# inferrna/Core

Hardware: AMD Instinct MI355X
Metric: Mrays/s (primary+shadow), 1M-tri scene (higher is better)
Workload: dtype f32

## Files before the change

core_amd/csrc/yk_device.hip:

```cpp
#include <hip/hip_runtime.h>

#include <algorithm>
#include <atomic>
#include <climits>
#include <chrono>
#include <cmath>
#include <cstdio>
#include <cstdlib>
#include <cstring>
#include <mutex>
#include <type_traits>
#include <stdexcept>
#include <string>
#include <thread>
#include <vector>

#include "../../include/yk_api.h"
#include "../../include/yk_test_hooks.h"
#include "../../include/yk_test_hooks_light.h"
#include "../../include/yk_test_hooks_camera.h"
#include "../../include/yk_test_hooks_film.h"
#include "../../include/yk_test_hooks_depth.h"
#include "photon_map.h"
#include "scene.h"
// ... 2665 lines not shown
          B.scol_next[3 * c + 1] = sc.g;
          B.scol_next[3 * c + 2] = sc.b;
          ps |= PS_CONT;
        }
      }
      B.pstate[c] = ps;
    }
  }
  unsigned sbase, qn;
  wave_append2<YK_BOUNCE_APPEND_WAVE>(qword, valid ? (unsigned)nr : 0u, emit_next ? 1u : 0u, sbase, qn);
  if (valid) flush_shadow(B, c, kend, nr, sbase + qpre, traced);
  if (emit_next) {
    st_ray(&B.q_rays[qin ^ 1][qn], nxt);
    B.q_owner[qin ^ 1][qn] = (int)c;
  }
}

inline auto shade_primary_fn(bool diff, bool xl, bool ao) {
  if (ao)
    return xl ? (diff ? k_shade_primary<true, true, true> : k_shade_primary<false, true, true>)
              : (diff ? k_shade_primary<true, false, true> : k_shade_primary<false, false, true>);
  return xl ? (diff ? k_shade_primary<true, true, false> : k_shade_primary<false, true, false>)
            : (diff ? k_shade_primary<true, false, false> : k_shade_primary<false, false, false>);
}
inline auto shade_bounce_fn(bool diff, bool xl) {
  return xl ? (diff ? k_shade_bounce<true, true> : k_shade_bounce<false, true>)
            : (diff ? k_shade_bounce<true, false> : k_shade_bounce<false, false>);
}

__global__ void __launch_bounds__(256) k_resolve_bounce(Batch B, RenderConst R,
                                                        const unsigned long long* __restrict__ qin_word, int depth,
                                                        int qin) {
  const long long nq = (long long)(*qin_word >> 32);
  const long long qi = (long long)blockIdx.x * blockDim.x + threadIdx.x;
  if (qi >= nq) return;
  const long long c = B.q_owner[qin][qi];
  const int ps = B.pstate[c];
  if (!(ps & PS_RESOLVE)) return;
  c3 lcol = C3(0.f, 0.f, 0.f);
  if (ps & PS_EST) {
    const int lnum = R.nlights > 1 ? B.lsel[c] : 0;
    lcol = cscale((float)R.nlights, resolve_light(B, c, 0, lnum));
  }
  if ((depth == 1 || R.spec) && (ps & PS_EMIT))
    lcol = cadd(lcol, C3(B.emit_b[3 * c], B.emit_b[3 * c + 1], B.emit_b[3 * c + 2]));
  const c3 thr = C3(B.thr[3 * c], B.thr[3 * c + 1], B.thr[3 * c + 2]);
  B.pathcol[3 * c] = B.pathcol[3 * c] + lcol.r * thr.r;
  B.pathcol[3 * c + 1] = B.pathcol[3 * c + 1] + lcol.g * thr.g;
  B.pathcol[3 * c + 2] = B.pathcol[3 * c + 2] + lcol.b * thr.b;
  if (ps & PS_CONT) {
    B.thr[3 * c] = thr.r * B.scol_next[3 * c];
    B.thr[3 * c + 1] = thr.g * B.scol_next[3 * c + 1];
    B.thr[3 * c + 2] = thr.b * B.scol_next[3 * c + 2];
    B.pstate[c] = PS_ALIVE;
  } else {
    B.pstate[c] = 0;
  }
}


__host__ __device__ inline Batch merged_region(Batch B, int depth) {
  B.slot_base = (long long)depth * B.cap;
  B.mq_region = depth;
  if (depth >= 1) {
    const long long o = (long long)(depth - 1) * B.cap;
    B.pstate += o;
    B.lsel += o;
    B.emit_b += 3 * o;
    B.scol_next += 3 * o;
  }
  return B;
}

__global__ void __launch_bounds__(256) k_resolve_merged(Batch B, RenderConst R, long long nc, int bounces) {
  const long long c = (long long)blockIdx.x * blockDim.x + threadIdx.x;
  if (c >= nc) return;
  c3 col = C3(B.col[3 * c], B.col[3 * c + 1], B.col[3 * c + 2]);
  if (!(B.prim_hit[c] & PH_DIFFUSE)) {
    B.samples[c] = make_float4(col.r, col.g, col.b, B.alpha[c]);
    return;
  }
  {
    c3 dl = C3(0.f, 0.f, 0.f);
    int k0 = 0;
    for (int l = 0; l < R.nlights; ++l) {
      dl = cadd(dl, resolve_light(B, c, k0, l));
      k0 += c_lights[l].nslots;
    }
    col = C3(col.r + dl.r, col.g + dl.g, col.b + dl.b);
  }
  c3 thr = C3(B.thr[3 * c], B.thr[3 * c + 1], B.thr[3 * c + 2]);
  c3 pc = C3(0.f, 0.f, 0.f);
  for (int depth = 1; depth <= bounces; ++depth) {
    const Batch Bd = merged_region(B, depth);
    const int ps = Bd.pstate[c];
    if (!(ps & PS_RESOLVE)) break;
    c3 lcol = C3(0.f, 0.f, 0.f);
    if (ps & PS_EST) {
      const int lnum = R.nlights > 1 ? Bd.lsel[c] : 0;
      lcol = cscale((float)R.nlights, resolve_light(Bd, c, 0, lnum));
    }
    if (depth == 1 && (ps & PS_EMIT))
      lcol = cadd(lcol, C3(Bd.emit_b[3 * c], Bd.emit_b[3 * c + 1], Bd.emit_b[3 * c + 2]));
    pc = C3(pc.r + lcol.r * thr.r, pc.g + lcol.g * thr.g, pc.b + lcol.b * thr.b);
    if (!(ps & PS_CONT)) break;
    thr = C3(thr.r * Bd.scol_next[3 * c], thr.g * Bd.scol_next[3 * c + 1], thr.b * Bd.scol_next[3 * c + 2]);
  }
  const float ns = (float)R.nsub;
  col = cadd(col, C3(pc.r / ns, pc.g / ns, pc.b / ns));
  B.samples[c] = make_float4(col.r, col.g, col.b, B.alpha[c]);
}

__global__ void __launch_bounds__(256) k_finish(Batch B, RenderConst R, long long nc) {
  const long long c = (long long)blockIdx.x * blockDim.x + threadIdx.x;
  if (c >= nc) return;
  c3 col = C3(B.col[3 * c], B.col[3 * c + 1], B.col[3 * c + 2]);
  if (R.integrator == YK_INTEGRATOR_PATH && (B.prim_hit[c] & PH_DIFFUSE)) {
    const float ns = (float)R.nsub;
    col = cadd(col, C3(B.pathcol[3 * c] / ns, B.pathcol[3 * c + 1] / ns, B.pathcol[3 * c + 2] / ns));
  }
  B.samples[c] = make_float4(col.r, col.g, col.b, B.alpha[c]);
}


enum : int { NF_HIT = 1, NF_LIGHT = 2, NF_LOOP = 4, NF_LOOPT = 8, NF_SPEC = 16 };

struct NodeStore {
  float* E;
  float* D;
  float* P;
  int* flags;
  int* child;
  float* rcol;
  float* alpha;
  yk_ray* ray;
  unsigned* soffs;
  unsigned* psample;
  unsigned long long* count;
  long long cap;
  int* overflow;
  float* malpha;
};

__global__ void __launch_bounds__(256) k_finish_spec(Batch B, RenderConst R, NodeStore NS, long long base,
                                                     long long n) {
  const long long i = (long long)blockIdx.x * blockDim.x + threadIdx.x;
  if (i >= n) return;
  const long long node = base + i;
  const int ph = B.prim_hit[i];
  const bool loop = R.integrator == YK_INTEGRATOR_PATH && (ph & PH_DIFFUSE);
  c3 P = C3(0.f, 0.f, 0.f);
  if (loop) {
    const float ns = (float)R.nsub;
    P = C3(B.pathcol[3 * i] / ns, B.pathcol[3 * i + 1] / ns, B.pathcol[3 * i + 2] / ns);
  }
  int f = 0;
  if (ph & PH_HIT) f |= NF_HIT;
  if (ph & PH_LIGHT) f |= NF_LIGHT;
  if (loop) f |= NF_LOOP | (B.incl[i] ? NF_LOOPT : 0);
  NS.flags[node] = f;
#pragma unroll
  for (int k = 0; k < 3; ++k) {
    NS.E[3 * node + k] = (ph & PH_HIT) ? B.emit0[3 * i + k] : 0.f;
    NS.D[3 * node + k] = B.col[3 * i + k];
  }
  NS.P[3 * node] = P.r;
  NS.P[3 * node + 1] = P.g;
  NS.P[3 * node + 2] = P.b;
  NS.child[2 * node] = -1;
  NS.child[2 * node + 1] = -1;
  NS.malpha[node] = 1.f;
  if (R.level == 0) NS.alpha[node] = B.alpha[i];
}

__global__ void __launch_bounds__(256) k_spawn(DScene S, Batch B, RenderConst R, NodeStore NS, long long base,
                                               long long n) {
  const long long i = (long long)blockIdx.x * blockDim.x + threadIdx.x;
  if (i >= n || !(B.prim_hit[i] & PH_HIT)) return;
  const int lv = R.level + 1;
  if (lv > R.rdepth || lv >= 20) return;
  const yk_hit h = B.p_hits[i];
  const yk_ray r = B.p_rays[i];
  const v3 from = V3(r.from[0], r.from[1], r.from[2]), dir = V3(r.dir[0], r.dir[1], r.dir[2]);
  const SurfPt sp = make_surface(S, from, dir, h);
  const DMat& M = c_mats[sp.mat];
  if (!(M.flags & (BSDF_SPECULAR | BSDF_FILTER))) return;
  const long long node = base + i;
  NS.flags[node] |= NF_SPEC;
  if (R.integrator == YK_INTEGRATOR_PHOTON && (M.flags & BSDF_FILTER)) {
    const v3 wo = vneg(dir);
    const float Kr = mat_fresnel(M, wo, face_forward(sp.Ng, sp.N, wo));
    const float refl = (1.f - M.comp[0] * Kr) * M.comp[1];
    NS.malpha[node] = 1.f - refl;
  }
  bool refl, refr;
  v3 d[2];
  c3 col[2];
  mat_specular(M, sp, vneg(dir), refl, refr, d, col);
  const bool want[2] = {refl, refr};
#pragma unroll
  for (int k = 0; k < 2; ++k) {
    if (!want[k]) continue;
    const unsigned long long id = atomicAdd(NS.count, 1ull);
    if ((long long)id >= NS.cap) {
      *NS.overflow = 1;
      continue;
    }
    NS.child[2 * node + k] = (int)id;
    NS.rcol[6 * node + 3 * k] = col[k].r;
    NS.rcol[6 * node + 3 * k + 1] = col[k].g;
    NS.rcol[6 * node + 3 * k + 2] = col[k].b;
    put_ray(NS.ray[id], sp.P, d[k], YK_MIN_RAYDIST, -1.0f);
    NS.soffs[id] = B.soffs[i];
    NS.psample[id] = B.psample[i];
  }
}

__global__ void __launch_bounds__(256) k_fold(Batch B, RenderConst R, NodeStore NS, long long nc) {
  const long long c = (long long)blockIdx.x * blockDim.x + threadIdx.x;
  if (c >= nc) return;
  constexpr int kMaxLevel = 22;
  int nodes[kMaxLevel], stage[kMaxLevel];
  c3 acc[kMaxLevel];
  float alp[kMaxLevel];
  const bool pt = R.integrator == YK_INTEGRATOR_PATH, pm = R.integrator == YK_INTEGRATOR_PHOTON;
  const float a_init = R.transp_bg ? 0.f : 1.f;
  float result_alpha = 0.f;
  bool e = true;
  int dd = 0;
  nodes[0] = (int)c;
  stage[0] = 0;
  c3 result = C3(0.f, 0.f, 0.f);
  for (;;) {
    const int n = nodes[dd];
    const int F = NS.flags[n];
    if (stage[dd] == 0) {
      c3 col = C3(NS.D[3 * n], NS.D[3 * n + 1], NS.D[3 * n + 2]);
      if (F & NF_HIT) {
        if (dd == 0) e = true;
        const bool incl = pt ? e : true;
        const c3 E = ((F & NF_LIGHT) && !incl) ? C3(0.f, 0.f, 0.f)
                                               : C3(NS.E[3 * n], NS.E[3 * n + 1], NS.E[3 * n + 2]);
        col = cadd(E, col);
        col = cadd(col, C3(NS.P[3 * n], NS.P[3 * n + 1], NS.P[3 * n + 2]));
        if (pt && (F & NF_LOOP)) e = (F & NF_LOOPT) != 0;
        if (F & NF_SPEC) e = true;
      }
      acc[dd] = col;
      alp[dd] = a_init;
      stage[dd] = 1;
      const int ch = (F & NF_HIT) ? NS.child[2 * n] : -1;
      if (ch >= 0 && dd + 1 < kMaxLevel) {
        ++dd;
        nodes[dd] = ch;
        stage[dd] = 0;
        continue;
      }
    }
    if (stage[dd] == 1) {
      stage[dd] = 2;
      const int ch = (F & NF_HIT) ? NS.child[2 * n + 1] : -1;
      if (ch >= 0 && dd + 1 < kMaxLevel) {
        ++dd;
        nodes[dd] = ch;
        stage[dd] = 0;
        continue;
      }
    }
    const c3 v = acc[dd];
    const float m = NS.malpha[n];
    const float va = (F & NF_HIT) ? m + (1.f - m) * alp[dd] : a_init;
    if (dd == 0) {
      result = v;
      result_alpha = va;
      break;
    }
    --dd;
    const int pn = nodes[dd];
    const int k = stage[dd] - 1;
    if (k == 1) alp[dd] = va;
    const float* rc = NS.rcol + 6 * pn + 3 * k;
    acc[dd] = cadd(acc[dd], C3(v.r * rc[0], v.g * rc[1], v.b * rc[2]));
  }
  B.samples[c] = make_float4(result.r, result.g, result.b, pm ? result_alpha : NS.alpha[c]);
}


struct FilmConst {
  int cx0, cy0, cx1, cy1, w, h;
  int tile, ntx;
  float filterw;
  double tableScale;
  int olo_x, ohi_x, olo_y, ohi_y;
  int shard, nshards;
  int tb0, tb1;
  const int* rank_of;
  int spp;
  float d1;
  const int* pmap;
  float table[256];
};

__device__ __forceinline__ int round2int(double v) { return (int)(v + (0.5 - 1.4e-11)); }
constexpr int kGatherGroup = 8;
__device__ __forceinline__ int floor2int(double v) { return (int)floor(v); }

__global__ void __launch_bounds__(256) k_pixel_extent(FilmConst F, const float2* __restrict__ sxy,
                                                      char4* __restrict__ ext, long long npix) {
  const long long slot = ((long long)blockIdx.x * blockDim.x + threadIdx.x) >> 6;
  const int lane = threadIdx.x & 63;
  if (slot >= npix) return;
  int x0 = 127, x1 = -128, y0 = 127, y1 = -128;
  for (int s = lane; s < F.spp; s += 64) {
    const float2 d = sxy[slot * F.spp + s];
    const double dx = d.x, dy = d.y;
    x0 = min(x0, round2int(dx - F.filterw));
    x1 = max(x1, round2int(dx + F.filterw - 1.0));
    y0 = min(y0, round2int(dy - F.filterw));
    y1 = max(y1, round2int(dy + F.filterw - 1.0));
  }
#pragma unroll
  for (int off = 32; off > 0; off >>= 1) {
    x0 = min(x0, __shfl_xor(x0, off));
    x1 = max(x1, __shfl_xor(x1, off));
    y0 = min(y0, __shfl_xor(y0, off));
    y1 = max(y1, __shfl_xor(y1, off));
  }
  if (lane == 0) ext[slot] = make_char4((signed char)x0, (signed char)x1, (signed char)y0, (signed char)y1);
}

template <bool CLAMP, bool PREMULT>
struct GatherColour {
  using Sample = float4;
  static constexpr bool kPremult = PREMULT;
  static constexpr int kStride = 5;
  float aR, aG, aB, aA, aW;
  __device__ __forceinline__ void load(const float* px) {
    aR = px[0];
    aG = px[1];
    aB = px[2];
    aA = px[3];
    aW = px[4];
  }
  __device__ __forceinline__ void store(float* px) const {
    px[0] = aR;
    px[1] = aG;
    px[2] = aB;
    px[3] = aA;
    px[4] = aW;
  }
  static __device__ __forceinline__ Sample none() { return make_float4(0.f, 0.f, 0.f, 0.f); }
  static __device__ __forceinline__ Sample fetch(const Sample* __restrict__ s, long long i) {
    float4 c = s[i];
    if constexpr (CLAMP) {
      c.x = c.x < 0.f ? 0.f : (c.x > 1.f ? 1.f : c.x);
      c.y = c.y < 0.f ? 0.f : (c.y > 1.f ? 1.f : c.y);
      c.z = c.z < 0.f ? 0.f : (c.z > 1.f ? 1.f : c.z);
    }
    return c;
  }
  __device__ __forceinline__ bool add(float wt, Sample c, int m) {
    if constexpr (PREMULT) {
      for (int i = 0; i < m; ++i) {
        c.x = c.x * c.w;
        c.y = c.y * c.w;
        c.z = c.z * c.w;
      }
    }
    aR = aR + wt * c.x;
    aG = aG + wt * c.y;
    aB = aB + wt * c.z;
    aA = aA + wt * c.w;
    aW = aW + wt;
    return true;
  }
};

struct GatherDepth {
  using Sample = float;
  static constexpr bool kPremult = false;
  static constexpr int kStride = 2;
  float aV, aW;
  __device__ __forceinline__ void load(const float* px) {
    aV = px[0];
    aW = px[1];
  }
  __device__ __forceinline__ void store(float* px) const {
    px[0] = aV;
    px[1] = aW;
  }
  static __device__ __forceinline__ Sample none() { return 0.f; }
  static __device__ __forceinline__ Sample fetch(const Sample* __restrict__ s, long long i) { return s[i]; }
  __device__ __forceinline__ bool add(float wt, Sample v, int) {
    if (v != v) return false;
    aV = aV + wt * v;
    aW = aW + wt;
    return true;
  }
};

template <class Acc>
__device__ __forceinline__ void film_gather_walk(const FilmConst& F, const typename Acc::Sample* __restrict__ samples,
                                                 const float2* __restrict__ sxy, const int* __restrict__ tile_base,
                                                 const char4* __restrict__ ext, float* __restrict__ film, int rx0,
                                                 int ry0, int rw, int rh) {
  const int tid = blockIdx.x * blockDim.x + threadIdx.x;
  if (tid >= rw * rh) return;
  const int tx = rx0 + tid % rw, ty = ry0 + tid / rw;
  if (tx < F.cx0 || tx >= F.cx1 || ty < F.cy0 || ty >= F.cy1) return;
  const int sx0 = max(F.cx0, tx - F.ohi_x), sx1 = min(F.cx1 - 1, tx - F.olo_x);
  const int sy0 = max(F.cy0, ty - F.ohi_y), sy1 = min(F.cy1 - 1, ty - F.olo_y);
  if (sx0 > sx1 || sy0 > sy1) return;
  const int tc0 = (sx0 - F.cx0) / F.tile, tc1 = (sx1 - F.cx0) / F.tile;
  const int tr0 = (sy0 - F.cy0) / F.tile, tr1 = (sy1 - F.cy0) / F.tile;
  float* px = film + Acc::kStride * ((size_t)(ty - F.cy0) * F.w + (tx - F.cx0));
  Acc a;
  a.load(px);
  bool any = false;
  auto tile = [&](int tr, int tc, int rank) {
      const int X = F.cx0 + tc * F.tile, Y = F.cy0 + tr * F.tile;
      const int W = min(F.tile, F.cx1 - X);
      const int ya = max(sy0, Y), yb = min(sy1, Y + F.tile - 1);
      const int xa = max(sx0, X), xb = min(sx1, X + F.tile - 1);
      const long long tb = tile_base[rank - F.tb0];
      for (int sy = ya; sy <= yb; ++sy)
        for (int sx = xa; sx <= xb; ++sx) {
          long long cbase;
          if (F.pmap) {
            cbase = F.pmap[(size_t)(sy - F.cy0) * F.w + (sx - F.cx0)];
            if (cbase < 0) continue;
          } else {
            cbase = tb + (long long)((sy - Y) * W + (sx - X)) * F.spp;
          }
          const int ox = tx - sx, oy = ty - sy;
          {
            const char4 e = ext[cbase / F.spp];
            if (ox < e.x || ox > e.y || oy < e.z || oy > e.w) continue;
          }
          for (int s0 = 0; s0 < F.spp; s0 += kGatherGroup) {
            float2 dd[kGatherGroup];
#pragma unroll
            for (int k = 0; k < kGatherGroup; ++k)
              dd[k] = (s0 + k < F.spp) ? sxy[cbase + s0 + k] : make_float2(-8.f, -8.f);
            float wt[kGatherGroup];
            bool acc[kGatherGroup];
            int mm[Acc::kPremult ? kGatherGroup : 1];
#pragma unroll
            for (int k = 0; k < kGatherGroup; ++k) {
              const double dx = dd[k].x, dy = dd[k].y;
              const int dx0 = round2int(dx - F.filterw), dx1 = round2int(dx + F.filterw - 1.0);
              const int dy0 = round2int(dy - F.filterw), dy1 = round2int(dy + F.filterw - 1.0);
              acc[k] = s0 + k < F.spp && !(ox < dx0 || ox > dx1 || oy < dy0 || oy > dy1);
              wt[k] = 0.f;
              if (acc[k]) {
                const int xi = floor2int(fabs(((double)ox - (dx - 0.5)) * F.tableScale));
                const int yi = floor2int(fabs(((double)oy - (dy - 0.5)) * F.tableScale));
                wt[k] = F.table[yi * 16 + xi];
                if constexpr (Acc::kPremult) {
                  const int wx0 = max(F.cx0 - sx, dx0), wx1 = min(F.cx1 - sx - 1, dx1);
                  const int wy0 = max(F.cy0 - sy, dy0);
                  mm[k] = (oy - wy0) * (wx1 - wx0 + 1) + (ox - wx0) + 1;
                }
              }
            }
            typename Acc::Sample col[kGatherGroup];
#pragma unroll
            for (int k = 0; k < kGatherGroup; ++k)
              col[k] = acc[k] ? Acc::fetch(samples, cbase + s0 + k) : Acc::none();
#pragma unroll
            for (int k = 0; k < kGatherGroup; ++k) {
              if (!acc[k]) continue;
              if (a.add(wt[k], col[k], Acc::kPremult ? mm[k] : 0)) any = true;
            }
          }
        }
  };
  if (F.rank_of) {
    int last = -1;
    for (;;) {
      int best = INT_MAX, btr = 0, btc = 0;
      for (int r = tr0; r <= tr1; ++r)
        for (int q = tc0; q <= tc1; ++q) {
          const int k = F.rank_of[r * F.ntx + q];
          if (k > last && k >= F.tb0 && k < F.tb1 && k < best) {
            best = k;
            btr = r;
            btc = q;
          }
        }
      if (best == INT_MAX) break;
      last = best;
      tile(btr, btc, best);
    }
  } else {
    for (int tr = tr0; tr <= tr1; ++tr)
      for (int tc = tc0; tc <= tc1; ++tc) {
        const int ti = tr * F.ntx + tc;
        if (ti % F.nshards != F.shard) continue;
        const int rank = ti / F.nshards;
        if (rank < F.tb0 || rank >= F.tb1) continue;
        tile(tr, tc, rank);
      }
  }
  if (!any) return;
  a.store(px);
}

template <bool CLAMP, bool PREMULT>
__global__ void __launch_bounds__(256) k_film_gather(FilmConst F, const float4* __restrict__ samples,
                                                     const float2* __restrict__ sxy, const int* __restrict__ tile_base,
                                                     const char4* __restrict__ ext, float* __restrict__ film,
                                                     int rx0, int ry0, int rw, int rh) {
  film_gather_walk<GatherColour<CLAMP, PREMULT>>(F, samples, sxy, tile_base, ext, film, rx0, ry0, rw, rh);
}

__global__ void __launch_bounds__(256) k_depth_gather(FilmConst F, const float* __restrict__ depths,
                                                      const float2* __restrict__ sxy, const int* __restrict__ tile_base,
                                                      const char4* __restrict__ ext, float* __restrict__ film,
                                                      int rx0, int ry0, int rw, int rh) {
  film_gather_walk<GatherDepth>(F, depths, sxy, tile_base, ext, film, rx0, ry0, rw, rh);
}

struct DepthConst {
  int normalize;
  float dmin, dinv;
};
__global__ void __launch_bounds__(256) k_depth_samples(const yk_ray* __restrict__ rays,
                                                       const yk_hit* __restrict__ hits, float* __restrict__ out,
                                                       DepthConst D, long long nc) {
  const long long c = (long long)blockIdx.x * blockDim.x + threadIdx.x;
  if (c >= nc) return;
  const yk_ray r = rays[c];
  const yk_hit h = hits[c];
  float depth;
  if (r.dir[0] == 0.f && r.dir[1] == 0.f && r.dir[2] == 0.f && r.tmin == 0.f && r.tmax == -1.0f) {
    depth = __int_as_float(0x7fc00000);
  } else {
    const float tmax = h.prim >= 0 ? h.t : r.tmax;
    if (D.normalize) {
      depth = 0.f;
      if (tmax > 0.f) depth = 1.f - (tmax - D.dmin) * D.dinv;
    } else {
      depth = tmax;
      if (depth <= 0.f) depth = 99999997952.f;
    }
  }
  out[c] = depth;
}

template <int KIND>
__global__ void __launch_bounds__(256) k_depth_range_rays(int resx, int resy, yk_ray* __restrict__ rays) {
  const long long t = (long long)blockIdx.x * blockDim.x + threadIdx.x;
  if (t >= (long long)resx * resy) return;
  const int i = (int)(t / resx), j = (int)(t % resx);
  yk_ray r;
  cam_shoot<KIND>((float)i, (float)j, 0.5f, 0.5f, r);
  rays[t] = r;
}

__global__ void __launch_bounds__(256) k_depth_range_reduce(const yk_ray* __restrict__ rays,
                                                            const yk_hit* __restrict__ hits, long long n,
                                                            unsigned* __restrict__ mm) {
  const long long t = (long long)blockIdx.x * blockDim.x + threadIdx.x;
  unsigned hi = 0u, lo = 0xFFFFFFFFu;
  if (t < n) {
    const yk_hit h = hits[t];
    float tmax = h.prim >= 0 ? h.t : rays[t].tmax;
    if (tmax == 0.f) tmax = 0.f;
    if (tmax >= 0.f) hi = lo = (unsigned)__float_as_int(tmax);
  }
#pragma unroll
  for (int off = 32; off > 0; off >>= 1) {
    hi = max(hi, (unsigned)__shfl_xor((int)hi, off));
    lo = min(lo, (unsigned)__shfl_xor((int)lo, off));
  }
  if ((threadIdx.x & 63) == 0) {
    if (hi != 0u) atomicMax(mm, hi);
    if (lo != 0xFFFFFFFFu) atomicMin(mm + 1, lo);
  }
}

constexpr int kMaxMultiDev = 16;
struct FilmShards {
  const float* f[kMaxMultiDev];
  int n;
};
__global__ void __launch_bounds__(256) k_film_sum(float* __restrict__ acc, FilmShards S, long long n) {
  const long long i4 = ((long long)blockIdx.x * blockDim.x + threadIdx.x) * 4;
  if (i4 >= n) return;
  if (i4 + 4 <= n) {
    float4 a = *reinterpret_cast<const float4*>(S.f[0] + i4);
    for (int k = 1; k < S.n; ++k) {
      const float4 b = *reinterpret_cast<const float4*>(S.f[k] + i4);
      a = make_float4(a.x + b.x, a.y + b.y, a.z + b.z, a.w + b.w);
    }
    *reinterpret_cast<float4*>(acc + i4) = a;
    return;
  }
  for (long long i = i4; i < n; ++i) {
    float a = S.f[0][i];
    for (int k = 1; k < S.n; ++k) a = a + S.f[k][i];
    acc[i] = a;
  }
}

__global__ void k_aa_flags(const float* __restrict__ film, int w, int h, float thr, uint8_t* __restrict__ flags) {
  const int tid = blockIdx.x * blockDim.x + threadIdx.x;
  if (tid >= (w - 1) * (h - 1)) return;
  const int x = tid % (w - 1), y = tid / (w - 1);
  const float* a = film + 5 * ((size_t)y * w + x);
  float c = 0.f;
  if (a[4] > 0.f) {
    const float inv = 1.0f / a[4];
    c = (0.2126f * fabsf(a[0] * inv) + 0.7152f * fabsf(a[1] * inv)) + 0.0722f * fabsf(a[2] * inv);
  }
  auto differs = [&](int nx, int ny) {
    const float* b = film + 5 * ((size_t)ny * w + nx);
    float d = c;
    if (b[4] > 0.f) {
      const float inv = 1.0f / b[4];
      d = (c - (0.0722f * b[2]) * inv) - (0.2126f * b[0] + 0.7152f * b[1]) * inv;
    }
    return fabsf(d) >= thr;
  };
  bool need = false;
  if (differs(x + 1, y)) { need = true; flags[(size_t)y * w + x + 1] = 1; }
  if (differs(x, y + 1)) { need = true; flags[(size_t)(y + 1) * w + x] = 1; }
  if (differs(x + 1, y + 1)) { need = true; flags[(size_t)(y + 1) * w + x + 1] = 1; }
  if (x > 0 && differs(x - 1, y + 1)) { need = true; flags[(size_t)(y + 1) * w + x - 1] = 1; }
  if (need) flags[(size_t)y * w + x] = 1;
}

__global__ void k_film_resolve(const float* __restrict__ film, float* __restrict__ rgba, long long npx, int premult) {
  const long long p = (long long)blockIdx.x * blockDim.x + threadIdx.x;
  if (p >= npx) return;
  const float* a = film + 5 * p;
  float r = 0.f, g = 0.f, b = 0.f, al = 0.f;
  if (a[4] > 0.f) {
    const float f = (float)(1.0 / (double)a[4]);
    r = a[0] * f;
    g = a[1] * f;
    b = a[2] * f;
    al = a[3] * f;
  }
  r = r < 0.f ? 0.f : r;
  g = g < 0.f ? 0.f : g;
  b = b < 0.f ? 0.f : b;
  if (premult) {
    r = r * al;
    g = g * al;
    b = b * al;
  }
  rgba[4 * p] = r;
  rgba[4 * p + 1] = g;
  rgba[4 * p + 2] = b;
  rgba[4 * p + 3] = al;
}

__global__ void k_depth_resolve(const float* __restrict__ depth, float* __restrict__ z, long long npx) {
  const long long p = (long long)blockIdx.x * blockDim.x + threadIdx.x;
  if (p >= npx) return;
  const float v = depth[2 * p], w = depth[2 * p + 1];
  z[p] = w > 0.f ? v / w : 0.f;
}

#include "yk_photon.inc"

}


using namespace yk;

#define HIPCHK(x)                                                                                \
  do {                                                                                           \
    hipError_t e_ = (x);                                                                         \
    if (e_ != hipSuccess)                                                                        \
      throw std::runtime_error(std::string("HIP error ") + hipGetErrorString(e_) + " at " #x); \
  } while (0)

namespace {

template <class T>
struct DBuf {
  T* p = nullptr;
  size_t n = 0;
  void ensure(size_t cnt) {
    if (cnt <= n && p) return;
    if (p) HIPCHK(hipFree(p));
    p = nullptr;
    n = 0;
    if (cnt == 0) return;
    HIPCHK(hipMalloc(&p, cnt * sizeof(T)));
    n = cnt;
  }
  void release() {
    if (p) (void)hipFree(p);
    p = nullptr;
    n = 0;
  }
  DBuf() = default;
  DBuf(const DBuf&) = delete;
  DBuf& operator=(const DBuf&) = delete;
  ~DBuf() { release(); }
};

template <class... KArgs, class... Args>
void launch(void (*kernel)(KArgs...), dim3 grid, dim3 block, size_t lds_bytes, hipStream_t stream, Args&&... args) {
  hipLaunchKernelGGL(kernel, grid, block, lds_bytes, stream, std::forward<Args>(args)...);
  HIPCHK(hipGetLastError());
}

}

struct Pipe {
  hipStream_t stream = nullptr;
  hipEvent_t ev0 = nullptr, ev1 = nullptr;
  DBuf<unsigned long long> counters;
  DBuf<unsigned long long> words;
  DBuf<uint2> ovf;
  std::vector<hipEvent_t> evpool;
  DBuf<unsigned> soffs, s_idx;
  DBuf<float> col, alpha, thr, pathcol, scol_next, wlast, emit_b, sl_contrib;
  DBuf<int> prim_hit, pstate, lsel, qo0, qo1, tile_base;
  DBuf<int4> tiles;
  DBuf<yk_ray> p_rays, qr0, qr1;
  DBuf<float4> s_dir;
  DBuf<yk_hit> p_hits, qh0, qh1;
  DBuf<uint8_t> sl_flags, s_occl;
  DBuf<float4> samples;
  DBuf<float2> sxy;
  DBuf<char4> pext;
  DBuf<unsigned> psample;
  DBuf<uint8_t> incl, caus;
  DBuf<float> emit0;
  DBuf<float> fgl, fglen;
  DBuf<float4> lkq;
  DBuf<float> s_filt, sl_aux;
  DBuf<float> zs;
  void create() {
    HIPCHK(hipStreamCreateWithFlags(&stream, hipStreamNonBlocking));
    HIPCHK(hipEventCreate(&ev0));
    HIPCHK(hipEventCreate(&ev1));
    counters.ensure(144);
  }
  hipEvent_t event(size_t i) {
    while (evpool.size() <= i) {
      hipEvent_t e;
      HIPCHK(hipEventCreate(&e));
      evpool.push_back(e);
    }
    return evpool[i];
  }
  ~Pipe() {
    for (auto e : evpool) (void)hipEventDestroy(e);
    if (ev0) (void)hipEventDestroy(ev0);
    if (ev1) (void)hipEventDestroy(ev1);
    if (stream) (void)hipStreamDestroy(stream);
  }
  template <class T>
  static long long held(const DBuf<T>& b) { return (long long)(b.n * sizeof(T)); }
  long long batch_bytes() const {
    return held(soffs) + held(s_idx) + held(col) + held(alpha) + held(thr) + held(pathcol) + held(scol_next) +
           held(wlast) + held(emit_b) + held(sl_contrib) + held(prim_hit) + held(pstate) + held(lsel) + held(qo0) +
           held(qo1) + held(tile_base) + held(tiles) + held(p_rays) + held(qr0) + held(qr1) + held(s_dir) +
           held(p_hits) + held(qh0) + held(qh1) + held(sl_flags) + held(s_occl) + held(samples) + held(sxy) +
           held(pext) + held(psample) + held(incl) + held(caus) + held(emit0) + held(fgl) + held(fglen) + held(lkq) +
           held(s_filt) + held(sl_aux) + held(zs);
  }
  long long all_bytes() const { return batch_bytes() + held(counters) + held(words) + held(ovf); }
  Batch bind(long long maxc, int K, int tiles_per_batch, bool spec, bool ts, int regions, bool split) {
    const long long nst = std::max(1, regions - 1);
    soffs.ensure(maxc);
    col.ensure(3 * maxc);
    alpha.ensure(maxc);
    prim_hit.ensure(maxc);
    p_rays.ensure(maxc);
    p_hits.ensure(maxc);
    thr.ensure(3 * maxc);
    pathcol.ensure(3 * maxc);
    scol_next.ensure(3 * maxc * nst);
    wlast.ensure(maxc);
    emit_b.ensure(3 * maxc * nst);
    pstate.ensure(maxc * nst);
    lsel.ensure(maxc * nst);
    qo0.ensure(maxc);
    qo1.ensure(maxc);
    qr0.ensure(maxc);
    qr1.ensure(maxc);
    qh0.ensure(maxc);
    qh1.ensure(maxc);
    s_dir.ensure(maxc * (split ? K + 1 : 2 * K) * regions);
    s_occl.ensure(maxc * K * regions);
    s_idx.ensure(maxc * K * regions);
    sl_contrib.ensure(3 * maxc * K * regions);
    sl_flags.ensure(maxc * K * regions);
    samples.ensure(maxc);
    sxy.ensure(maxc);
    pext.ensure(maxc);
    tiles.ensure(tiles_per_batch);
    tile_base.ensure(tiles_per_batch + 1);
    Batch B{};
    B.prim_hit = prim_hit.p;
    B.soffs = soffs.p;
    B.col = col.p;
    B.alpha = alpha.p;
    B.p_rays = p_rays.p;
    B.p_hits = p_hits.p;
// ... 1091 lines not shown
```

core_amd/csrc/yk_render_host.inc:

```
struct PassSpec {
  int n, off;
  bool multipass;
  const uint8_t* flags;
  float* d_depth = nullptr;
};

namespace {

bool needs_photon_maps(const yk_render_params* p) {
  return p->integrator == YK_INTEGRATOR_PHOTON ||
         (p->integrator == YK_INTEGRATOR_PATH &&
          (p->caustic_type == YK_CAUSTIC_PHOTON || p->caustic_type == YK_CAUSTIC_BOTH)) ||
         (p->integrator == YK_INTEGRATOR_DIRECT && p->dl_caustics != 0);
}

int check_tiles(const yk_render_params* p) {
  const int tile = p->tile_size > 0 ? p->tile_size : 32;
  if (tile > 4096) return set_error(YK_ERR_UNSUPPORTED, "tile_size > 4096");
  const int ntiles = ((p->width + tile - 1) / tile) * ((p->height + tile - 1) / tile);
  if (ntiles >= (1 << 19)) return set_error(YK_ERR_UNSUPPORTED, "too many tiles");
  if (p->tile_order && p->tile_order_len > 0) {
    if (p->tile_order_len != ntiles)
      return set_error(YK_ERR_ARG, "tile_order must list every tile of the render area once");
    std::vector<char> seen((size_t)ntiles, 0);
    for (int i = 0; i < ntiles; ++i) {
      const int t = p->tile_order[i];
      if (t < 0 || t >= ntiles || seen[(size_t)t])
        return set_error(YK_ERR_ARG, "tile_order is not a permutation of the tiles");
      seen[(size_t)t] = 1;
    }
  }
  return YK_OK;
}

int check_depth_params(const yk_render_params* p) {
  if (!p->z_channel) return YK_OK;
  if (!p->depth_film) return set_error(YK_ERR_ARG, "z_channel needs a depth_film");
  if (p->normalize_z_channel && !std::isfinite(p->depth_min))
    return set_error(YK_ERR_ARG, "normalize_z_channel needs a finite depth_min (yk_depth_range)");
  return YK_OK;
}

int check_render_params(const yk_device* d, const yk_render_params* p, int32_t shard, int32_t nshards,
                        const float* d_film, const PassSpec& ps) {
  if (!d || !p || !d_film || nshards < 1 || shard < 0 || shard >= nshards)
    return set_error(YK_ERR_ARG, "yk_render_shard: bad arguments");
  if (!d->uploaded) return set_error(YK_ERR_STATE, "yk_render_shard: no scene uploaded");
  if (p->filter < YK_FILTER_BOX || p->filter > YK_FILTER_LANCZOS) return set_error(YK_ERR_ARG, "unknown filter");
  if (p->integrator != YK_INTEGRATOR_PATH && p->integrator != YK_INTEGRATOR_DIRECT &&
      p->integrator != YK_INTEGRATOR_PHOTON)
    return set_error(YK_ERR_ARG, "unknown integrator");
  if (p->integrator == YK_INTEGRATOR_PATH &&
      (p->caustic_type < YK_CAUSTIC_NONE || p->caustic_type > YK_CAUSTIC_BOTH))
    return set_error(YK_ERR_ARG, "unknown caustic_type");
  if (needs_photon_maps(p) && (!d->pm_ready || d->pm_integrator != p->integrator))
    return set_error(YK_ERR_STATE, "photon maps: call yk_photon_build for this integrator first (preprocess)");
  if (needs_photon_maps(p) && std::memcmp(&p->photon, &d->pm_params, sizeof(yk_photon_params)) != 0)
    return set_error(YK_ERR_STATE, "photon mapping: the maps were built with different photon parameters");
  const bool ao = p->integrator == YK_INTEGRATOR_DIRECT && p->do_ao != 0;
  if (ao && p->ao_samples < 1) return set_error(YK_ERR_ARG, "AO_samples must be >= 1");
  if (ao && !(std::isfinite(p->ao_distance) && p->ao_distance > 0.f))
    return set_error(YK_ERR_ARG, "AO_distance must be finite and > 0");
  if (ao && (long long)d->sum_light_slots + p->ao_samples > 8192)
    return set_error(YK_ERR_UNSUPPORTED,
                     "too many shadow slots per shading point (light samples + AO_samples > 8192)");
  if (p->integrator == YK_INTEGRATOR_PATH && (p->bounces < 1 || 4 * p->bounces + 4 >= 50))
    return set_error(YK_ERR_UNSUPPORTED, "bounces must be in [1, 11]");
  if (p->width <= 0 || p->height <= 0) return set_error(YK_ERR_ARG, "empty render area");
  if (p->filter_width != 0.f && !(p->filter_width >= 0.501f && p->filter_width <= 4.f))
    return set_error(YK_ERR_ARG, "filter_width must be 0 or in [0.501, 4]");
  if (const int rc = check_tiles(p)) return rc;
  if (p->transp_shadows && (p->shadow_depth < 0 || p->shadow_depth > 8))
    return set_error(YK_ERR_UNSUPPORTED, "shadowDepth must be in [0, 8] with transpShad");
  if (ps.flags && (p->xstart + p->width > 65535 || p->ystart + p->height > 65535))
    return set_error(YK_ERR_UNSUPPORTED, "adaptive passes need coordinates < 65536");
  if (const int rc = check_depth_params(p)) return rc;
  return YK_OK;
}

struct TileLists {
  std::vector<int> owned;
  std::vector<int> rank_of;
  std::vector<int4> tiles, rect_of;
  std::vector<int> base;
  std::vector<long long> nc_of;
  std::vector<int> pix, pmap;
  std::vector<size_t> pix_off;
};

void owned_tiles(const FilmConst& F, const int32_t* tile_order, int tile_order_len, TileLists& L) {
  const int ntiles = F.ntx * ((F.h + F.tile - 1) / F.tile);
  if (tile_order && tile_order_len > 0) {
    L.rank_of.assign((size_t)ntiles, -1);
    for (int i = 0; i < ntiles; ++i) {
      const int t = tile_order[i];
      if (t % F.nshards != F.shard) continue;
      L.rank_of[(size_t)t] = (int)L.owned.size();
      L.owned.push_back(t);
    }
  } else {
    for (int t = F.shard; t < ntiles; t += F.nshards) L.owned.push_back(t);
  }
}

void build_tile_lists(const FilmConst& F, int nbatch, int tpb, int spp, const uint8_t* flags, TileLists& L) {
  L.base.assign((size_t)nbatch * (tpb + 1), 0);
  L.nc_of.assign(nbatch, 0);
  L.rect_of.resize(nbatch);
  L.pix_off.assign(nbatch, 0);
  if (flags) L.pmap.assign((size_t)F.w * F.h, -1);
  for (int bi = 0; bi < nbatch; ++bi) {
    const size_t tb0 = (size_t)bi * tpb, tb1 = std::min(L.owned.size(), tb0 + (size_t)tpb);
    long long nc = 0;
    int rx0 = 1 << 30, ry0 = 1 << 30, rx1 = -(1 << 30), ry1 = -(1 << 30);
    L.pix_off[bi] = L.pix.size();
    for (size_t k = tb0; k < tb1; ++k) {
      const int t = L.owned[k];
      const int X = F.cx0 + (t % F.ntx) * F.tile, Y = F.cy0 + (t / F.ntx) * F.tile;
      const int W = std::min(F.tile, F.cx1 - X), H = std::min(F.tile, F.cy1 - Y);
      L.tiles.push_back(make_int4(X, Y, W, H));
      L.base[(size_t)bi * (tpb + 1) + (k - tb0)] = (int)nc;
      if (flags) {
        for (int yy = Y; yy < Y + H; ++yy)
          for (int xx = X; xx < X + W; ++xx) {
            const size_t px = (size_t)(yy - F.cy0) * F.w + (xx - F.cx0);
            if (!flags[px]) continue;
            L.pmap[px] = (int)nc;
            L.pix.push_back((yy << 16) | xx);
            nc += spp;
          }
      } else {
        nc += (long long)W * H * spp;
      }
      rx0 = std::min(rx0, X);
      ry0 = std::min(ry0, Y);
      rx1 = std::max(rx1, X + W);
      ry1 = std::max(ry1, Y + H);
    }
    L.base[(size_t)bi * (tpb + 1) + (tb1 - tb0)] = (int)nc;
    L.nc_of[bi] = nc;
    L.rect_of[bi] = make_int4(rx0, ry0, rx1, ry1);
  }
}

struct FilmOptions {
  bool clamp, premult;
};
inline FilmOptions film_options(const yk_render_params* p) { return FilmOptions{p->clamp_rgb != 0, p->premult_alpha != 0}; }
void launch_film_gather(hipStream_t stream, const FilmConst& F, const int* pmap, int tb0, int tb1, int4 rect,
                        long long nc, const float4* samples, const float2* sxy, const int* base, char4* pext,
                        float* d_film, FilmOptions opt = FilmOptions{false, false}, const float* depths = nullptr,
                        float* d_depth = nullptr) {
  FilmConst Fb = F;
  Fb.pmap = pmap;
  Fb.tb0 = tb0;
  Fb.tb1 = tb1;
  const int gx0 = std::max(F.cx0, rect.x + F.olo_x), gy0 = std::max(F.cy0, rect.y + F.olo_y);
  const int gx1 = std::min(F.cx1, rect.z + F.ohi_x), gy1 = std::min(F.cy1, rect.w + F.ohi_y);
  const int gw = gx1 - gx0, gh = gy1 - gy0;
  if (nc > 0 && gw > 0 && gh > 0) {
    const long long npix = nc / F.spp;
    launch(k_pixel_extent, grid_for(npix * 64), 256, 0, stream, Fb, sxy, pext, npix);
    auto* gather = opt.clamp ? (opt.premult ? k_film_gather<true, true> : k_film_gather<true, false>)
                             : (opt.premult ? k_film_gather<false, true> : k_film_gather<false, false>);
    if (samples)
      launch(gather, grid_for((long long)gw * gh), 256, 0, stream, Fb, samples, sxy, base, pext, d_film, gx0, gy0, gw,
             gh);
    if (depths)
      launch(k_depth_gather, grid_for((long long)gw * gh), 256, 0, stream, Fb, depths, sxy, base, pext, d_depth, gx0,
             gy0, gw, gh);
  }
}

struct FramePlan : TileLists {
  bool pm, cmap, ao, path, merged, split;
  FilmConst F;
  RenderConst R;
  AOConst AOC;
  PMConst PMC;
  int K;
  int bounces, nsub;
  int spec_levels;
  yk_batch_plan plan;
  int qwords_per_batch, launches_per_batch;
  long long words_per_batch;
};

const char* build_frame_plan(const yk_device* d, const yk_render_params* p, int32_t shard, int32_t nshards,
                             const PassSpec& ps, FramePlan& fp) {
  fp.pm = p->integrator == YK_INTEGRATOR_PHOTON;
  fp.path = p->integrator == YK_INTEGRATOR_PATH;
  const bool pt_cmap = fp.path && (p->caustic_type == YK_CAUSTIC_PHOTON || p->caustic_type == YK_CAUSTIC_BOTH);
  fp.cmap = needs_photon_maps(p) && !fp.pm;
  fp.ao = p->integrator == YK_INTEGRATOR_DIRECT && p->do_ao != 0;
  FilmConst& F = fp.F;
  F = make_film(p);
  F.shard = shard;
  F.nshards = nshards;
  F.spp = ps.n;
  F.d1 = (float)(1.0 / (double)(float)ps.n);
  F.rank_of = nullptr;
  const int spp = F.spp;
  owned_tiles(F, p->tile_order, p->tile_order_len, fp);
  RenderConst& R = fp.R;
  R = RenderConst{};
  R.spp = spp;
  R.nsub = fp.path ? std::max(1, p->path_samples) : 1;
  R.pm_fg = (fp.pm && p->photon.final_gather && !p->photon.show_map) ? 1 : 0;
  R.pm_showmap = (fp.pm && p->photon.show_map) ? 1 : 0;
  if (R.pm_fg) R.nsub = std::max(1, p->photon.fg_samples);
  fp.PMC = needs_photon_maps(p) ? pm_const(d, p->photon) : PMConst{};
  R.bounces = p->bounces;
  R.integrator = p->integrator;
  R.transp_bg = p->transp_background;
  R.nlights = d->nlights;
  R.has_bg = d->has_bg ? 1 : 0;
  for (int k = 0; k < 3; ++k) R.bg[k] = d->bg[k];
  R.d1 = F.d1;
  R.spec = d->spec ? 1 : 0;
  R.trace_caustics =
      (fp.path && (p->caustic_type == YK_CAUSTIC_PATH || p->caustic_type == YK_CAUSTIC_BOTH)) ? 1 : 0;
  R.rdepth = p->raydepth;
  R.level = 0;
  R.multipass = ps.multipass ? 1 : 0;
  R.pass_off = ps.off;
  R.ps = (R.spec || R.multipass) ? 1 : 0;
  fp.K = std::max(1, d->sum_light_slots + ao_slots(p));
  fp.AOC = AOConst{};
  if (fp.ao) {
    fp.AOC.n = p->ao_samples;
    fp.AOC.k0 = d->sum_light_slots;
    fp.AOC.dist = p->ao_distance;
    for (int k = 0; k < 3; ++k) fp.AOC.col[k] = p->ao_color[k];
  }
  fp.spec_levels = d->spec ? std::max(0, std::min(p->raydepth, 19)) : 0;
  const char* merge_env = std::getenv("YK_MERGE");
  fp.merged = !(merge_env && std::atoi(merge_env) == 0) && fp.path && !d->spec && !pt_cmap && !p->transp_shadows &&
              p->path_samples <= 1 && p->bounces >= 1;
  R.merged = fp.merged ? 1 : 0;
  static const long long batch_gb_env = [] {
    const char* e = std::getenv("YK_BATCH_GB");
    const long long v = e ? std::atoll(e) : 0;
    return (v > 0 && v <= 240) ? v : 0ll;
  }();
  fp.split = shadow_split(d, p);
  yk_batch_plan_in pin{};
  pin.slots = fp.K;
  pin.bounces = fp.merged ? p->bounces : 0;
  pin.merged = fp.merged ? 1 : 0;
  pin.split = fp.split ? 1 : 0;
  pin.transp_shadows = p->transp_shadows ? 1 : 0;
  pin.spec = d->spec ? 1 : 0;
  pin.final_gather = R.pm_fg;
  pin.spec_levels = fp.spec_levels;
  pin.tile = F.tile;
  pin.spp = spp;
  pin.pipes = pipes_env();
  pin.reserved = p->z_channel ? 1 : 0;
  pin.owned_tiles = (long long)fp.owned.size();
  const char* target_env = std::getenv("YK_BATCH_SAMPLES");
  pin.target_samples = target_env ? std::atoll(target_env) : 0;
  pin.budget_bytes = (batch_gb_env ? batch_gb_env : (fp.merged ? 192ll : 64ll)) << 30;
  if (const char* why = plan_batches(pin, fp.plan)) return why;
  fp.bounces = fp.path ? R.bounces : (R.pm_fg ? p->photon.fg_bounces + 1 : 0);
  fp.nsub = (fp.path || R.pm_fg) ? R.nsub : 1;
  fp.qwords_per_batch = fp.nsub * (fp.bounces + 1);
  fp.launches_per_batch = 2 + 2 * fp.nsub * fp.bounces + (R.pm_fg ? fp.nsub * fp.bounces : 0);
  fp.words_per_batch = 2ll * fp.qwords_per_batch + 128ll * fp.launches_per_batch;

  build_tile_lists(F, fp.plan.nbatch, fp.plan.tiles_per_batch, spp, ps.flags, fp);
  return nullptr;
}

void upload_frame_plan(yk_device* d, FramePlan& fp) {
  auto up = [](auto& dev, const auto& host, size_t at_least) {
    dev.ensure(std::max(at_least, host.size()));
    if (!host.empty())
      HIPCHK(hipMemcpy(dev.p, host.data(), host.size() * sizeof(host[0]), hipMemcpyHostToDevice));
  };
  up(d->tiles_dev, fp.tiles, 0);
  up(d->base_dev, fp.base, 0);
  if (!fp.pmap.empty()) {
    up(d->pix_dev, fp.pix, 1);
    up(d->pmap_dev, fp.pmap, 0);
  }
  if (!fp.rank_of.empty()) {
    up(d->rank_dev, fp.rank_of, 0);
    fp.F.rank_of = d->rank_dev.p;
  }
}

void bind_pipes(yk_device* d, const yk_render_params* p, const FramePlan& fp, Batch* Bp) {
  const yk_batch_plan& pl = fp.plan;
  for (int pi = 0; pi < pl.npipes; ++pi) {
    Pipe& P = d->pipe[pi];
    const int nb_here = (pl.nbatch - pi + pl.npipes - 1) / pl.npipes;
    P.words.ensure((size_t)(2 * kAccWords + (d->spec ? 0 : fp.words_per_batch * nb_here)));
    HIPCHK(hipMemsetAsync(P.words.p, 0, P.words.n * sizeof(unsigned long long), P.stream));
    Bp[pi] = P.bind(pl.maxc, fp.K, pl.tiles_per_batch, fp.R.ps != 0, p->transp_shadows != 0, pl.regions, fp.split);
    if (p->z_channel) P.zs.ensure(pl.maxc);
    if (fp.R.pm_fg) {
      P.fgl.ensure(3 * pl.maxc);
      P.fglen.ensure(pl.maxc);
      P.lkq.ensure(2 * pl.maxc);
    }
  }
}

NodeStore bind_node_store(yk_device* d, const FramePlan& fp) {
  if (!d->spec) return NodeStore{};
  const long long cap = fp.plan.maxc * ((2ll << fp.spec_levels) - 1);
  d->nE.ensure(3 * cap);
  d->nD.ensure(3 * cap);
  d->nP.ensure(3 * cap);
  d->nrcol.ensure(6 * cap);
  d->nalpha.ensure(fp.plan.maxc);
  d->nflags.ensure(cap);
  d->nchild.ensure(2 * cap);
  d->nray.ensure(cap);
  d->nsoffs.ensure(cap);
  d->npsample.ensure(cap);
  d->ncount.ensure(1);
  d->noverflow.ensure(1);
  d->nmalpha.ensure(cap);
  d->spec_words.ensure((size_t)fp.words_per_batch);
  HIPCHK(hipMemsetAsync(d->noverflow.p, 0, sizeof(int), d->pipe[0].stream));
  return NodeStore{d->nE.p,   d->nD.p,     d->nP.p,       d->nflags.p, d->nchild.p,    d->nrcol.p,    d->nalpha.p,
                   d->nray.p, d->nsoffs.p, d->npsample.p, d->ncount.p, (long long)cap, d->noverflow.p, d->nmalpha.p};
}

struct Timed {
  int pipe;
  size_t ev;
  bool closest;
};

bool cam_can_die(const yk_device* d) { return d->cam_host.kind == YK_CAMERA_ANGULAR && d->cam_host.circular != 0; }

struct BatchCtx {
  yk_device* d;
  const yk_render_params* p;
  const FramePlan* fp;
  const PassSpec* ps;
  float* d_film;
  NodeStore NS;
  std::vector<Timed>* timed;
  size_t* evn;
  int pi;
  Pipe* P;
  Batch B;
  unsigned long long* bw;
  int launch;
  unsigned long long* live = nullptr;
  float* zs = nullptr;
  DepthConst DC{};
};

unsigned long long* qw(const BatchCtx& c, int isub, int depth) { return c.bw + isub * (c.fp->bounces + 1) + depth; }
unsigned long long* next_work(BatchCtx& c) { return c.bw + 2ll * c.fp->qwords_per_batch + 128ll * c.launch++; }

void trace(BatchCtx& c, bool closest, RaySrc rays, const unsigned* idx, RayCount n, yk_hit* hits, uint8_t* occ) {
  Pipe& P = *c.P;
  unsigned long long* work = next_work(c);
  const hipEvent_t e0 = P.event(c.evn[c.pi]), e1 = P.event(c.evn[c.pi] + 1);
  c.timed->push_back(Timed{c.pi, c.evn[c.pi], closest});
  c.evn[c.pi] += 2;
  if (closest) enqueue_trace<true>(c.d, P, rays, idx, n, hits, occ, work, P.words.p, e0, e1);
  else if (c.B.ts)
    enqueue_trace_ts(c.d, P, rays, idx, n, occ, c.B.s_filt, c.p->shadow_depth, work, P.words.p + kAccWords, e0, e1);
  else enqueue_trace<false>(c.d, P, rays, idx, n, hits, occ, work, P.words.p + kAccWords, e0, e1);
}
void trace_shadow_slots(BatchCtx& c, const Batch& Bc, RayCount n) {
  trace(c, false, shadow_src(Bc), Bc.s_idx, n, nullptr, Bc.s_occl);
}

void enqueue_photon_mapping(BatchCtx& c, const Batch& Bc, const RenderConst& Rc, long long n) {
  yk_device* d = c.d;
  Pipe& P = *c.P;
  const PMConst& PMC = c.fp->PMC;
  const int fg_bounces = c.p->photon.fg_bounces;
  if (PMC.show_map || !PMC.final_gather) launch(k_pm_post, grid_for(n, 64), 64, 0, P.stream, d->S, Bc, PMC, n);
  for (int isub = 0; isub < (Rc.pm_fg ? c.fp->nsub : 0); ++isub) {
    launch(d->diff_only ? k_fg_start<true> : k_fg_start<false>, grid_for(n, YK_APPEND_BLOCK), YK_APPEND_BLOCK, 0,
           P.stream, d->S, Bc, Rc, n, isub, P.fgl.p, qw(c, isub, 0));
    int qin = 1;
    for (int it = 0; it <= fg_bounces; ++it) {
      const unsigned long long* in_w = qw(c, isub, it);
      unsigned long long* out_w = qw(c, isub, it + 1);
      trace(c, true, ray_src(Bc.q_rays[qin]), nullptr, RayCount{in_w, 32, 0}, Bc.q_hits[qin], nullptr);
      unsigned long long* lk_w = qw(c, isub, it) + c.fp->qwords_per_batch;
      launch(d->diff_only ? k_fg_hit<true> : k_fg_hit<false>, grid_for(n, YK_APPEND_BLOCK), YK_APPEND_BLOCK, 0,
             P.stream, d->S, Bc, Rc, PMC, in_w, it, isub, qin, P.fgl.p, P.fglen.p, out_w, P.lkq.p, lk_w);
      if (it < fg_bounces) trace_shadow_slots(c, Bc, RayCount{out_w, 0, 0});
      const bool lds = lookup_lds(d);
      launch(lds ? k_pm_lookup<true> : k_pm_lookup<false>, (unsigned)((long long)d->cus * d->per_cu_lookup[lds]), 64,
             lds ? lookup_lds_bytes(d->rm_depth) : 0, P.stream, PMC.rmap, PMC.lookup_rad, d->rm_depth, P.lkq.p, lk_w,
             P.fgl.p, next_work(c));
      launch(k_fg_resolve, grid_for(n), 256, 0, P.stream, Bc, Rc, in_w, qin, P.fgl.p);
      qin ^= 1;
    }
  }
  launch(k_pm_finish, grid_for(n, 64), 64, 0, P.stream, d->S, Bc, Rc, PMC, n);
}

void enqueue_post_direct(BatchCtx& c, const Batch& Bc, const RenderConst& Rc, long long n) {
  const FramePlan& fp = *c.fp;
  hipStream_t s = c.P->stream;
  if (fp.pm) enqueue_photon_mapping(c, Bc, Rc, n);
  if (fp.cmap && fp.PMC.cmap.n != 0)
    launch(k_pt_caustic, grid_for(n, 64), 64, 0, s, c.d->S, Bc, fp.PMC, n);
  if (fp.ao) launch(k_resolve_ao, grid_for(n), 256, 0, s, c.d->S, Bc, Rc, fp.AOC, n);
}

void enqueue_entries(BatchCtx& c, const Batch& Bc, const RenderConst& Rc, long long n, long long node_base) {
  yk_device* d = c.d;
  const FramePlan& fp = *c.fp;
  hipStream_t s = c.P->stream;
  const bool merged = fp.merged;
  const bool post_direct_after_bounces = d->spec;
  if (d->spec) {
    HIPCHK(hipMemsetAsync(d->spec_words.p, 0, d->spec_words.n * sizeof(unsigned long long), s));
    c.launch = 0;
  }
  if (c.live && node_base == 0) trace(c, true, ray_src(Bc.p_rays), Bc.s_idx, RayCount{c.live, 0, 0}, Bc.p_hits, nullptr);
  else trace(c, true, ray_src(Bc.p_rays), nullptr, RayCount{nullptr, 0, n}, Bc.p_hits, nullptr);
  if (c.zs && node_base == 0) launch(k_depth_samples, grid_for(n), 256, 0, s, Bc.p_rays, Bc.p_hits, c.zs, c.DC, n);
  launch(shade_primary_fn(d->diff_only, d->xl_lights, fp.ao), grid_for(n, YK_PRIMARY_BLOCK), YK_PRIMARY_BLOCK, 0, s,
         d->S, Bc, Rc, n, qw(c, 0, 0), fp.AOC);
  if (!merged) {
    trace_shadow_slots(c, Bc, RayCount{qw(c, 0, 0), 0, 0});
    launch(k_resolve_primary, grid_for(n), 256, 0, s, Bc, Rc, n);
  }
  if (!post_direct_after_bounces) enqueue_post_direct(c, Bc, Rc, n);
  const int bblock = bounce_block(d->diff_only);
  for (int isub = 0; isub < (fp.path ? fp.nsub : 0); ++isub) {
    if (isub > 0)
      launch(d->diff_only ? k_path_start<true> : k_path_start<false>, grid_for(n, YK_BOUNCE_BLOCK), YK_BOUNCE_BLOCK, 0,
             s, d->S, Bc, Rc, n, isub, qw(c, isub, 0));
    int qin = 1;
    for (int depth = 1; depth <= fp.bounces; ++depth) {
      const unsigned long long* in_w = qw(c, isub, depth - 1);
      unsigned long long* out_w = qw(c, isub, depth);
      trace(c, true, ray_src(Bc.q_rays[qin]), nullptr, RayCount{in_w, 32, 0}, Bc.q_hits[qin], nullptr);
      Batch Bd = Bc;
      if (merged) {
        Bd = merged_region(Bc, depth);
        Bd.mq_words = qw(c, 0, 0);
      }
      launch(shade_bounce_fn(d->diff_only, d->xl_lights), grid_for(n, bblock), bblock, 0, s, d->S, Bd, Rc, in_w, depth,
             isub, qin, out_w);
      if (!merged) {
        trace_shadow_slots(c, Bc, RayCount{out_w, 0, 0});
        launch(k_resolve_bounce, grid_for(n), 256, 0, s, Bc, Rc, in_w, depth, qin);
      }
      qin ^= 1;
    }
  }
  if (post_direct_after_bounces) enqueue_post_direct(c, Bc, Rc, n);
  if (d->spec) {
    launch(k_finish_spec, grid_for(n), 256, 0, s, Bc, Rc, c.NS, node_base, n);
    launch(k_spawn, grid_for(n), 256, 0, s, d->S, Bc, Rc, c.NS, node_base, n);
  } else if (merged) {
    trace_shadow_slots(c, Bc, RayCount{qw(c, 0, 0), 0, 0, fp.plan.regions});
    launch(k_resolve_merged, grid_for(n), 256, 0, s, Bc, Rc, n, fp.bounces);
  } else {
    launch(k_finish, grid_for(n), 256, 0, s, Bc, Rc, n);
  }
}

int enqueue_spec_generations(BatchCtx& c, long long nc) {
  const FramePlan& fp = *c.fp;
  const NodeStore& NS = c.NS;
  hipStream_t s = c.P->stream;
// ... 461 lines not shown
```

Baseline: 3498.

## Split film gather samples across an 8-lane group per output pixel

The film and depth gather kernels now give each output pixel a group of 8 lanes instead of one thread. The lanes split each chunk of 16 samples: each lane loads its own sample positions, computes the filter weight and fetches the colour. Each lane then places its results in shared memory, and a ballot mask guides every lane in the group through the accepted samples in the original order, so the accumulation sequence is unchanged. The aim is more memory-level parallelism and fewer serial per-thread loads in the gather. In exchange it launches 8x more threads, adds LDS traffic and wave barriers, and repeats the accumulation on every lane of the group.

```diff
diff --git a/core_amd/csrc/yk_device.hip b/core_amd/csrc/yk_device.hip
--- a/core_amd/csrc/yk_device.hip
+++ b/core_amd/csrc/yk_device.hip
@@ -2991,7 +2991,6 @@
 };
 
 __device__ __forceinline__ int round2int(double v) { return (int)(v + (0.5 - 1.4e-11)); }
-constexpr int kGatherGroup = 8;
 __device__ __forceinline__ int floor2int(double v) { return (int)floor(v); }
 
 __global__ void __launch_bounds__(256) k_pixel_extent(FilmConst F, const float2* __restrict__ sxy,
@@ -3088,14 +3087,34 @@
   }
 };
 
+constexpr int kGatherLanes = 8;
+constexpr int kGatherChunk = 16;
+static_assert(kGatherLanes >= 1 && kGatherLanes <= 64 && (kGatherLanes & (kGatherLanes - 1)) == 0, "lane group");
+static_assert(kGatherChunk >= kGatherLanes && kGatherChunk % kGatherLanes == 0, "chunk");
+
+__device__ __forceinline__ void wave_lds_sync() {
+  __builtin_amdgcn_fence(__ATOMIC_RELEASE, "wavefront");
+  __builtin_amdgcn_wave_barrier();
+  __builtin_amdgcn_fence(__ATOMIC_ACQUIRE, "wavefront");
+}
+
 template <class Acc>
 __device__ __forceinline__ void film_gather_walk(const FilmConst& F, const typename Acc::Sample* __restrict__ samples,
                                                  const float2* __restrict__ sxy, const int* __restrict__ tile_base,
                                                  const char4* __restrict__ ext, float* __restrict__ film, int rx0,
                                                  int ry0, int rw, int rh) {
-  const int tid = blockIdx.x * blockDim.x + threadIdx.x;
-  if (tid >= rw * rh) return;
-  const int tx = rx0 + tid % rw, ty = ry0 + tid / rw;
+  constexpr int G = kGatherLanes, U = kGatherChunk / kGatherLanes;
+  constexpr unsigned long long gmask = G == 64 ? ~0ull : (1ull << (G & 63)) - 1ull;
+  __shared__ float s_wt[256];
+  __shared__ typename Acc::Sample s_col[256];
+  __shared__ int s_m[Acc::kPremult ? 256 : 1];
+  const long long gid = ((long long)blockIdx.x * blockDim.x + threadIdx.x) / G;
+  const int me = threadIdx.x;
+  const int gl = me % G;
+  const int gb = me - gl;
+  const int wl0 = gb & 63;
+  if (gid >= (long long)rw * rh) return;
+  const int tx = rx0 + (int)(gid % rw), ty = ry0 + (int)(gid / rw);
   if (tx < F.cx0 || tx >= F.cx1 || ty < F.cy0 || ty >= F.cy1) return;
   const int sx0 = max(F.cx0, tx - F.ohi_x), sx1 = min(F.cx1 - 1, tx - F.olo_x);
   const int sy0 = max(F.cy0, ty - F.ohi_y), sy1 = min(F.cy1 - 1, ty - F.olo_y);
@@ -3126,40 +3145,52 @@
             const char4 e = ext[cbase / F.spp];
             if (ox < e.x || ox > e.y || oy < e.z || oy > e.w) continue;
           }
-          for (int s0 = 0; s0 < F.spp; s0 += kGatherGroup) {
-            float2 dd[kGatherGroup];
+          for (int s0 = 0; s0 < F.spp; s0 += kGatherChunk) {
+            float2 dd[U];
 #pragma unroll
-            for (int k = 0; k < kGatherGroup; ++k)
-              dd[k] = (s0 + k < F.spp) ? sxy[cbase + s0 + k] : make_float2(-8.f, -8.f);
-            float wt[kGatherGroup];
-            bool acc[kGatherGroup];
-            int mm[Acc::kPremult ? kGatherGroup : 1];
+            for (int u = 0; u < U; ++u)
+              dd[u] = (s0 + u * G + gl < F.spp) ? sxy[cbase + s0 + u * G + gl] : make_float2(-8.f, -8.f);
+            float wt[U];
+            bool acc[U];
+            int mm[Acc::kPremult ? U : 1];
+            unsigned long long bits[U], some = 0;
 #pragma unroll
-            for (int k = 0; k < kGatherGroup; ++k) {
-              const double dx = dd[k].x, dy = dd[k].y;
+            for (int u = 0; u < U; ++u) {
+              const double dx = dd[u].x, dy = dd[u].y;
               const int dx0 = round2int(dx - F.filterw), dx1 = round2int(dx + F.filterw - 1.0);
               const int dy0 = round2int(dy - F.filterw), dy1 = round2int(dy + F.filterw - 1.0);
-              acc[k] = s0 + k < F.spp && !(ox < dx0 || ox > dx1 || oy < dy0 || oy > dy1);
-              wt[k] = 0.f;
-              if (acc[k]) {
+              acc[u] = s0 + u * G + gl < F.spp && !(ox < dx0 || ox > dx1 || oy < dy0 || oy > dy1);
+              wt[u] = 0.f;
+              if (acc[u]) {
                 const int xi = floor2int(fabs(((double)ox - (dx - 0.5)) * F.tableScale));
                 const int yi = floor2int(fabs(((double)oy - (dy - 0.5)) * F.tableScale));
-                wt[k] = F.table[yi * 16 + xi];
+                wt[u] = F.table[yi * 16 + xi];
                 if constexpr (Acc::kPremult) {
                   const int wx0 = max(F.cx0 - sx, dx0), wx1 = min(F.cx1 - sx - 1, dx1);
                   const int wy0 = max(F.cy0 - sy, dy0);
-                  mm[k] = (oy - wy0) * (wx1 - wx0 + 1) + (ox - wx0) + 1;
+                  mm[u] = (oy - wy0) * (wx1 - wx0 + 1) + (ox - wx0) + 1;
                 }
               }
+              bits[u] = (__ballot(acc[u]) >> wl0) & gmask;
+              some |= bits[u];
             }
-            typename Acc::Sample col[kGatherGroup];
+            if (!some) continue;
+            typename Acc::Sample col[U];
 #pragma unroll
-            for (int k = 0; k < kGatherGroup; ++k)
-              col[k] = acc[k] ? Acc::fetch(samples, cbase + s0 + k) : Acc::none();
+            for (int u = 0; u < U; ++u)
+              col[u] = acc[u] ? Acc::fetch(samples, cbase + s0 + u * G + gl) : Acc::none();
 #pragma unroll
-            for (int k = 0; k < kGatherGroup; ++k) {
-              if (!acc[k]) continue;
-              if (a.add(wt[k], col[k], Acc::kPremult ? mm[k] : 0)) any = true;
+            for (int u = 0; u < U; ++u) {
+              if (!bits[u]) continue;
+              s_wt[me] = wt[u];
+              s_col[me] = col[u];
+              if constexpr (Acc::kPremult) s_m[me] = mm[u];
+              wave_lds_sync();
+              for (unsigned long long b = bits[u]; b; b &= b - 1) {
+                const int k = gb + __ffsll((long long)b) - 1;
+                if (a.add(s_wt[k], s_col[k], Acc::kPremult ? s_m[k] : 0)) any = true;
+              }
+              wave_lds_sync();
             }
           }
         }
@@ -3191,7 +3222,7 @@
         tile(tr, tc, rank);
       }
   }
-  if (!any) return;
+  if (!any || gl != 0) return;
   a.store(px);
 }
 
diff --git a/core_amd/csrc/yk_render_host.inc b/core_amd/csrc/yk_render_host.inc
--- a/core_amd/csrc/yk_render_host.inc
+++ b/core_amd/csrc/yk_render_host.inc
@@ -164,11 +164,11 @@
     auto* gather = opt.clamp ? (opt.premult ? k_film_gather<true, true> : k_film_gather<true, false>)
                              : (opt.premult ? k_film_gather<false, true> : k_film_gather<false, false>);
     if (samples)
-      launch(gather, grid_for((long long)gw * gh), 256, 0, stream, Fb, samples, sxy, base, pext, d_film, gx0, gy0, gw,
-             gh);
+      launch(gather, grid_for((long long)gw * gh * kGatherLanes), 256, 0, stream, Fb, samples, sxy, base, pext, d_film,
+             gx0, gy0, gw, gh);
     if (depths)
-      launch(k_depth_gather, grid_for((long long)gw * gh), 256, 0, stream, Fb, depths, sxy, base, pext, d_depth, gx0,
-             gy0, gw, gh);
+      launch(k_depth_gather, grid_for((long long)gw * gh * kGatherLanes), 256, 0, stream, Fb, depths, sxy, base, pext,
+             d_depth, gx0, gy0, gw, gh);
   }
 }
 
```

After: 3522, median of 6. No clear change (+0.7%).
